# addtt/ladder-vae-pytorch

Hardware: AMD Instinct MI355X
Metric: training images/sec (ELBO step: fwd+bwd+Adamax) (higher is better)
Workload: dtype f32; 1 GPU; CIFAR10-shaped 15-layer LVAE (BASELINE configs[2]): 32x32x3, zdims 32x15, 4 blocks/layer, 64 filters, gated+skip, DMoL-10, dropout 0.2, free bits 1.0; batch_per_gpu=256, global_batch=256, parallelism=dp1, hip_graph=True

## Files before the change

ladder-vae-pytorch_amd/csrc/conv3x3_wino.hip:

```cpp
#include <stdlib.h>
#include <string.h>

#include "bf16_frag.h"
#include "bn_stats.h"
#include "lvae_host.h"

#ifndef LVAE_W1_RING
#define LVAE_W1_RING 3
#endif

namespace lvae {

struct WinoArgs {
  lvae_conv_desc d;
  const float* U;
  int TH, TW, NI, tiles_h, halo_w, halo_h, halo_px, ntn, Npad, tiles_x, wt_per_img, n_wt, Cin;
  uint32_t m_thw, m_per_img, m_halo_w, m_tiles_x, m_wt_per_img, m_tw;
  lvae_bn_fold f;
  int store_pivot;
  const __bf16* g_ws;
  const float* g_bias;
  const float* g_res;
  float* g_ab;
  float* g_out;
// ... 216 lines not shown
      const bool live = hoff[u] != ~0u && 16 * c + hc4 < a.Cin;
      const unsigned off = live ? hoff[u] + 16 * c : 0u;
      if (dbg & 1) hreg[u] = zero4;
      else hreg[u] = *reinterpret_cast<const f32x4*>(d.x + off);
      hlive = live ? hlive | (1u << u) : hlive & ~(1u << u);
    }
  };
  __shared__ __attribute__((aligned(16))) float s_coef[128];
  const bool folded = CIN == 64 && a.f.parts != nullptr;
  const bool bn_in = d.in_scale != nullptr || folded;
  auto store_slice = [&](int c) {
    f32x4 sc = {1.f, 1.f, 1.f, 1.f}, sh = zero4;
    if (bn_in && 16 * c + hc4 < a.Cin) {
      if (folded) {
        sc = *reinterpret_cast<const f32x4*>(s_coef + 16 * c + hc4);
        sh = *reinterpret_cast<const f32x4*>(s_coef + 64 + 16 * c + hc4);
      } else {
        sc = *reinterpret_cast<const f32x4*>(d.in_scale + 16 * c + hc4);
        sh = *reinterpret_cast<const f32x4*>(d.in_shift + 16 * c + hc4);
      }
    }
#pragma unroll
    for (int u = 0; u < SLOTS; ++u) {
      if (hlds[u] >= 0) {
        f32x4 w = zero4;
        if ((hlive >> u) & 1u) {
          w = hreg[u];
          if (bn_in) w = act_fwd4(w * sc + sh, d.in_act);
        }
        *reinterpret_cast<f32x4*>(As + hlds[u] + 16 * c) = w;
      }
    }
  };
  load_slice(0);

  const int ra = wave == 0 ? 0 : (wave == 2 ? 2 : 1);
  const int rb = wave == 0 ? 2 : (wave == 1 ? 2 : (wave == 2 ? 1 : 3));
  const float sgn = wave == 1 ? 1.f : -1.f;
  const float* pa[MT];
  const float* pb[MT];
#pragma unroll
  for (int m = 0; m < MT; ++m) {
    int wt = li + 32 * m;
    if (wt >= a.n_wt) wt = 0;
    const int wimg = fastdiv(wt, a.m_wt_per_img), wr = wt - wimg * a.wt_per_img;
    const int wty = fastdiv(wr, a.m_tiles_x), wtx = wr - wty * a.tiles_x;
    const int pbase = (wimg * a.halo_h + 2 * wty) * a.halo_w + 2 * wtx;
    pa[m] = As + (size_t)(pbase + ra * a.halo_w) * WLDA + (SPL ? 8 : 4) * lh;
    pb[m] = As + (size_t)(pbase + rb * a.halo_w) * WLDA + (SPL ? 8 : 4) * lh;
  }

  f32x16 acc[MT][4][NH];
#pragma unroll
  for (int m = 0; m < MT; ++m)
#pragma unroll
    for (int j = 0; j < 4; ++j)
#pragma unroll
      for (int h = 0; h < NH; ++h)
#pragma unroll
        for (int r = 0; r < 16; ++r) acc[m][j][h][r] = 0.f;

  if (folded) wino_fold_bn<256>(a.f, a.Cin, smem, s_coef, t, bid == 0);
  store_slice(0);
  load_slice(1);
  __syncthreads();
  WINO_STAMP(1);
  if (!SPL) {
    const size_t slab = (size_t)a.Npad * CIN;
    const float* ub = a.U + (size_t)(4 * wave) * slab + ((size_t)lh * a.Npad + co0 + li) * 4;
    const size_t kstep = (size_t)2 * a.Npad * 4;
    f32x4 bf[RING][4][NH];
    auto load_u = [&](int ks, int buf) {
  #pragma unroll
      for (int j = 0; j < 4; ++j)
  #pragma unroll
        for (int h = 0; h < NH; ++h) bf[buf][j][h] = *reinterpret_cast<const f32x4*>(ub + j * slab + ks * kstep + h * 128);
    };
  #pragma unroll
    for (int q = 0; q < RING - 1; ++q) load_u(q, q);

  #pragma unroll
    for (int ks = 0; ks < KSTEPS; ++ks) {
      if (ks + RING - 1 < KSTEPS) load_u(ks + RING - 1, (ks + RING - 1) % RING);
      if (NH == 1) __builtin_amdgcn_sched_barrier(0);
  #pragma unroll
      for (int m = 0; m < MT; ++m) {
        f32x4 tt[4];
  #pragma unroll
        for (int c = 0; c < 4; ++c) {
          const f32x4 da = *reinterpret_cast<const f32x4*>(pa[m] + c * WLDA + ks * 8);
          const f32x4 db = *reinterpret_cast<const f32x4*>(pb[m] + c * WLDA + ks * 8);
  #pragma unroll
          for (int e = 0; e < 4; ++e) tt[c][e] = __builtin_fmaf(sgn, db[e], da[e]);
        }
        f32x4 vv[4];
        vv[0] = tt[0] - tt[2];
        vv[1] = tt[1] + tt[2];
        vv[2] = tt[2] - tt[1];
        vv[3] = tt[1] - tt[3];
  #pragma unroll
        for (int j = 0; j < 4; ++j)
  #pragma unroll
          for (int h = 0; h < NH; ++h)
  #pragma unroll
            for (int e = 0; e < 4; ++e)
              acc[m][j][h] = __builtin_amdgcn_mfma_f32_32x32x2f32(vv[j][e], bf[ks % RING][j][h][e], acc[m][j][h], 0, 0, 0);
      }
      if (NH == 1) __builtin_amdgcn_sched_barrier(0);
      if ((ks & 1) && ks < KSTEPS - 1) {
        const int c = (ks + 1) >> 1;
        store_slice(c);
        if (c + 1 < NSLICE) load_slice(c + 1);
        __syncthreads();
      }
    }
  } else {
    const int NB = a.Npad >> 5;
    const __bf16* u3 = reinterpret_cast<const __bf16*>(a.U) + ((size_t)(co0 >> 5) * 3 * 64 + lane) * 8;
    constexpr int BR = LVAE_W1_RING;
    bf16x8 bq[BR][NH][3];
    auto load_b = [&](int it, int buf) {
      const __bf16* p = u3 + ((dbg & 8) ? (size_t)0 : (size_t)((4 * wave + (it & 3)) * 4 + (it >> 2)) * NB * 1536);
#pragma unroll
      for (int h = 0; h < NH; ++h)
#pragma unroll
        for (int q = 0; q < 3; ++q) bq[buf][h][q] = *reinterpret_cast<const bf16x8*>(p + (h * 3 + q) * 512);
    };
#pragma unroll
    for (int it = 0; it < (BR < 4 * NSLICE ? BR - 1 : BR); ++it) load_b(it, it);
#pragma unroll
    for (int s16 = 0; s16 < NSLICE; ++s16) {
      f32x4 tl[4], th[4];
      if (!(dbg & 2)) {
#pragma unroll
      for (int c = 0; c < 4; ++c) {
        const f32x4 dal = *reinterpret_cast<const f32x4*>(pa[0] + c * WLDA + s16 * 16);
        const f32x4 dah = *reinterpret_cast<const f32x4*>(pa[0] + c * WLDA + s16 * 16 + 4);
        const f32x4 dbl = *reinterpret_cast<const f32x4*>(pb[0] + c * WLDA + s16 * 16);
        const f32x4 dbh = *reinterpret_cast<const f32x4*>(pb[0] + c * WLDA + s16 * 16 + 4);
#pragma unroll
        for (int e = 0; e < 4; ++e) {
          tl[c][e] = __builtin_fmaf(sgn, dbl[e], dal[e]);
          th[c][e] = __builtin_fmaf(sgn, dbh[e], dah[e]);
        }
      }
#pragma unroll
      for (int j = 0; j < 4; ++j) {
        const int it = 4 * s16 + j;
        if (BR < 4 * NSLICE && it + BR - 1 < 4 * NSLICE) load_b(it + BR - 1, (it + BR - 1) % BR);
        const f32x4 vl = j == 0 ? tl[0] - tl[2] : (j == 1 ? tl[1] + tl[2] : (j == 2 ? tl[2] - tl[1] : tl[1] - tl[3]));
        const f32x4 vh = j == 0 ? th[0] - th[2] : (j == 1 ? th[1] + th[2] : (j == 2 ? th[2] - th[1] : th[1] - th[3]));
        bf16x8 af[3];
        if (dbg & 32) {
          af[0] = __builtin_bit_cast(bf16x8, vl);
          af[1] = __builtin_bit_cast(bf16x8, vh);
          af[2] = __builtin_bit_cast(bf16x8, vl + vh);
        } else {
        split_frag<3>(vl, vh, af);
        }
#pragma unroll
        for (int h = 0; h < NH; ++h) acc[0][j][h] = mfma_pieces<3>(af, bq[it % BR][h], acc[0][j][h]);
      }
      } else {
#pragma unroll
        for (int j = 0; j < 4; ++j) {
          const int it = 4 * s16 + j;
          if (BR < 4 * NSLICE && it + BR - 1 < 4 * NSLICE) load_b(it + BR - 1, (it + BR - 1) % BR);
#pragma unroll
          for (int h = 0; h < NH; ++h)
#pragma unroll
            for (int q = 0; q < 3; ++q) acc[0][j][h][q] += (float)bq[it % BR][h][q][0];
        }
      }
      if (s16 < NSLICE - 1) {
        store_slice(s16 + 1);
        if (s16 + 2 < NSLICE) load_slice(s16 + 2);
        __syncthreads();
      }
    }
  }
  WINO_STAMP(2);
  __syncthreads();
  WINO_STAMP(3);
  if (dbg & 16) {
    float keep = 0.f;
#pragma unroll
    for (int j = 0; j < 4; ++j)
#pragma unroll
      for (int h = 0; h < NH; ++h) keep += acc[0][j][h][j + h];
    if (keep == 12345.678f) d.y[t] = 1.f;
    return;
  }

  float* Rs = smem;
#pragma unroll
  for (int m = 0; m < MT; ++m)
#pragma unroll
    for (int h = 0; h < NH; ++h)
#pragma unroll
      for (int r = 0; r < 16; ++r) {
        const int tile = 32 * m + (r & 3) + 8 * (r >> 2) + 4 * lh;
        const float r0 = acc[m][0][h][r] + acc[m][1][h][r] + acc[m][2][h][r];
        const float r1 = acc[m][1][h][r] - acc[m][2][h][r] - acc[m][3][h][r];
        float* o = Rs + (size_t)((wave * 2) * NT + tile) * WLDO + h * 32 + li;
        o[0] = r0;
        o[NT * WLDO] = r1;
      }
  __syncthreads();
  WINO_STAMP(4);
  {
    const int c4 = (t % C4N) * 4, col = co0 + c4;
    f32x4 st1 = zero4, st2 = zero4, piv, bsh, bmu, brs;
    stats_load_coef4(d.stats_pivot, d.Cout, col, d.stats_out != nullptr, d.stats_mode == LVAE_STATS_BN_BWD, piv, bsh, bmu, brs);
    if (col < d.Cout) {
      f32x4 bias = zero4;
      if (d.bias) bias = *reinterpret_cast<const f32x4*>(d.bias + col);
      const int thw = a.TH * a.TW;
      const int nvalid = min(a.NI, d.N - n0) * thw;
      float* yb = d.y + ((size_t)(n0 * d.H + oh0) * d.W) * d.Cout + col;
#pragma unroll
      for (int q = 0; q < QN; ++q) {
        const int p = t / C4N + PG * q;
        if (p < nvalid) {
          const int img = fastdiv(p, a.m_thw), pr = p - img * thw;
          const int oy = fastdiv(pr, a.m_tw), ox = pr - oy * a.TW;
          const int tile = img * a.wt_per_img + (oy >> 1) * a.tiles_x + (ox >> 1);
          const float* rp = Rs + (size_t)((ox & 1) * NT + tile) * WLDO + c4;
          const f32x4 R0 = *reinterpret_cast<const f32x4*>(rp);
          const f32x4 R1 = *reinterpret_cast<const f32x4*>(rp + 2 * NT * WLDO);
          const f32x4 R2 = *reinterpret_cast<const f32x4*>(rp + 4 * NT * WLDO);
          const f32x4 R3 = *reinterpret_cast<const f32x4*>(rp + 6 * NT * WLDO);
          f32x4 v = (oy & 1) ? (R1 - R2 - R3) : (R0 + R1 + R2);
          v = v + bias;
          if (d.out_scale) v = v * *reinterpret_cast<const f32x4*>(d.out_scale + (size_t)(n0 + img) * d.Cout + col);
          v = act_fwd4(v, d.out_act);
          if (!(dbg & 4) || v[0] == 12345.678f) store_wt4(yb + (size_t)p * d.Cout, v);
          if (d.stats_mode == LVAE_STATS_BN_BWD) {
            if (d.stats_out) {
              const f32x4 xv = *reinterpret_cast<const f32x4*>(d.stats_x + (size_t)((n0 * d.H + oh0) * d.W + p) * d.Cout + col);
              stats_bwd_accum4(v, xv, piv, bsh, bmu, brs, d.stats_act, st1, st2);
            }
          } else {
            stats_fwd_accum4(v, piv, st1, st2);
          }
        }
      }
    }
    WINO_STAMP(5);
    if (d.stats_out)
      stats_reduce_groups<PG, CW>(smem, t / C4N, c4, st1, st2, d.stats_out, tm, d.Cout, co0, a.store_pivot && tm == 0, d.stats_pivot,
                                  gridDim.x / a.ntn);
  }
}


#ifndef LVAE_W2_PAIRSPLIT
#define LVAE_W2_PAIRSPLIT 1
#endif

constexpr int W2_LDS_R = 8 * 2 * 32 * WLDO * 4;

template <bool GATE>
__global__ __launch_bounds__(512) void conv3x3_wino2_kernel(WinoArgs a) {
  kernarg_warmup<sizeof(WinoArgs)>();
  constexpr int CIN = 64, WLDA = CIN + 4, NSLICE = CIN / 16, CW = 64, C4N = CW / 4, PG = 512 / C4N, NH = 2;
  extern __shared__ __attribute__((aligned(16))) float smem[];
  float* As = smem;
  const lvae_conv_desc& d = a.d;
  const int t = threadIdx.x, lane = t & 63, wave = __builtin_amdgcn_readfirstlane(t >> 6);
  const int li = lane & 31, lh = lane >> 5;
  const int prow = wave >> 1, jp = wave & 1;
  WINO_STAMP(0);
#ifdef LVAE_WINO_DBG
  constexpr int dbg = LVAE_WINO_DBG;
#else
  constexpr int dbg = 0;
#endif
  int bid = blockIdx.x;
  {
    const int nwg = gridDim.x, xcd = bid & 7, q = nwg >> 3, r = nwg & 7;
    bid = (xcd < r ? xcd * (q + 1) : r * (q + 1) + (xcd - r) * q) + (bid >> 3);
  }
  const int tile_n = bid % a.ntn;
  const int tm = bid / a.ntn;
  const int th_idx = tm % a.tiles_h, ig = tm / a.tiles_h;
  const int n0 = ig * a.NI, oh0 = th_idx * a.TH, co0 = tile_n * CW;
  const f32x4 zero4 = {0.f, 0.f, 0.f, 0.f};

  constexpr int SLOTS = 3;
  const int per_img = a.halo_h * a.halo_w;
  const int hc4 = (t & 3) * 4;
  unsigned hoff[SLOTS];
  int hlds[SLOTS];
#pragma unroll
  for (int u = 0; u < SLOTS; ++u) {
    const int px = (t >> 2) + 128 * u;
    const int img = fastdiv(px, a.m_per_img), r = px - img * per_img;
    const int hy = fastdiv(r, a.m_halo_w), hx = r - hy * a.halo_w;
    const int n = n0 + img, ih = oh0 + hy - 1, iw = hx - 1;
    const bool ok = (n < d.N) & ((unsigned)ih < (unsigned)d.H) & ((unsigned)iw < (unsigned)d.W) & (px < a.halo_px);
    hoff[u] = ok ? (unsigned)(((n * d.H + ih) * d.W + iw) * a.Cin + hc4) : ~0u;
    hlds[u] = px < a.halo_px ? px * WLDA + hc4 : a.halo_px * WLDA + 4 * t;
  }
  __shared__ __attribute__((aligned(16))) float s_coef[128];
  const bool folded = a.f.parts != nullptr;
  const bool bn_in = d.in_scale != nullptr || folded;
  f32x4 hreg[SLOTS];
  unsigned hlive = 0;
  auto load_slice = [&](int c) {
#pragma unroll
    for (int u = 0; u < SLOTS; ++u) {
      const bool live = hoff[u] != ~0u && 16 * c + hc4 < a.Cin;
      const unsigned off = live ? hoff[u] + 16 * c : 0u;
      if (dbg & 1) hreg[u] = zero4;
      else hreg[u] = *reinterpret_cast<const f32x4*>(d.x + off);
      hlive = live ? hlive | (1u << u) : hlive & ~(1u << u);
    }
  };
  auto store_slice = [&](int c) {
    if (bn_in) {
      const int cc = 16 * c + hc4 < a.Cin ? 16 * c + hc4 : 0;
      f32x4 sc, sh;
      if (folded) {
        sc = *reinterpret_cast<const f32x4*>(s_coef + cc);
        sh = *reinterpret_cast<const f32x4*>(s_coef + 64 + cc);
      } else {
        sc = *reinterpret_cast<const f32x4*>(d.in_scale + cc);
        sh = *reinterpret_cast<const f32x4*>(d.in_shift + cc);
      }
#pragma unroll
      for (int u = 0; u < SLOTS; ++u) {
        f32x4 w;
#pragma unroll
        for (int e = 0; e < 4; ++e) w[e] = hreg[u][e] * sc[e] + sh[e];
        w = act_fwd4(w, d.in_act);
        const bool live = (hlive >> u) & 1u;
#pragma unroll
        for (int e = 0; e < 4; ++e) w[e] = live ? w[e] : 0.f;
        *reinterpret_cast<f32x4*>(As + hlds[u] + 16 * c) = w;
      }
    } else {
#pragma unroll
      for (int u = 0; u < SLOTS; ++u) {
        f32x4 w = hreg[u];
        const bool live = (hlive >> u) & 1u;
#pragma unroll
        for (int e = 0; e < 4; ++e) w[e] = live ? w[e] : 0.f;
        *reinterpret_cast<f32x4*>(As + hlds[u] + 16 * c) = w;
      }
    }
  };
  load_slice(0);

  const int ra = prow == 0 ? 0 : (prow == 2 ? 2 : 1);
  const int rb = prow == 0 ? 2 : (prow == 1 ? 2 : (prow == 2 ? 1 : 3));
  const float sgn = prow == 1 ? 1.f : -1.f;
  const float s2 = jp ? -1.f : 1.f;
  const int col0 = jp ? 2 : 0, col1 = jp ? 1 : 2, col2 = jp ? 3 : 1;
  const float* pa[2];
  const float* pb[2];
#pragma unroll
  for (int m = 0; m < 2; ++m) {
    const int wt = li + 32 * m;
    const int wimg = fastdiv(wt, a.m_wt_per_img), wr = wt - wimg * a.wt_per_img;
    const int wty = fastdiv(wr, a.m_tiles_x), wtx = wr - wty * a.tiles_x;
    const int pbase = (wimg * a.halo_h + 2 * wty) * a.halo_w + 2 * wtx;
    pa[m] = As + (size_t)(pbase + ra * a.halo_w) * WLDA + 8 * lh;
    pb[m] = As + (size_t)(pbase + rb * a.halo_w) * WLDA + 8 * lh;
  }

  f32x16 acc[2][2][NH];
#pragma unroll
  for (int m = 0; m < 2; ++m)
#pragma unroll
    for (int j = 0; j < 2; ++j)
#pragma unroll
      for (int h = 0; h < NH; ++h)
#pragma unroll
        for (int r = 0; r < 16; ++r) acc[m][j][h][r] = 0.f;

  if (folded) wino_fold_bn<512>(a.f, a.Cin, smem, s_coef, t, bid == 0);
  store_slice(0);
  load_slice(1);
  __syncthreads();
  WINO_STAMP(1);
  {
    const int NB = a.Npad >> 5;
    const __bf16* u3 = reinterpret_cast<const __bf16*>(a.U) + ((size_t)(co0 >> 5) * 3 * 64 + lane) * 8;
#ifndef LVAE_W2_RING
#define LVAE_W2_RING 2
#endif
    constexpr int BR = LVAE_W2_RING, NIT = 2 * NSLICE;
    bf16x8 bq[BR][NH][3];
    auto load_b = [&](int it, int buf) {
      const __bf16* p = u3 + ((dbg & 8) ? (size_t)0 : (size_t)((4 * prow + 2 * jp + (it & 1)) * 4 + (it >> 1)) * NB * 1536);
#pragma unroll
      for (int h = 0; h < NH; ++h)
#pragma unroll
        for (int q = 0; q < 3; ++q) bq[buf][h][q] = *reinterpret_cast<const bf16x8*>(p + (h * 3 + q) * 512);
    };
#pragma unroll
    for (int it = 0; it < BR - 1; ++it) load_b(it, it);
    auto make_af = [&](const f32x4 (&tl)[2][3], const f32x4 (&th)[2][3], int jj, int m, bf16x8 (&af)[3]) {
      f32x4 vl, vh;
      if (jj == 0) {
#pragma unroll
        for (int e = 0; e < 4; ++e) {
          vl[e] = tl[m][0][e] - tl[m][1][e];
          vh[e] = th[m][0][e] - th[m][1][e];
        }
      } else {
#pragma unroll
        for (int e = 0; e < 4; ++e) {
          vl[e] = __builtin_fmaf(s2, tl[m][2][e], tl[m][1][e]);
          vh[e] = __builtin_fmaf(s2, th[m][2][e], th[m][1][e]);
        }
      }
      if (dbg & 32) {
        af[0] = __builtin_bit_cast(bf16x8, vl);
        af[1] = __builtin_bit_cast(bf16x8, vh);
        af[2] = __builtin_bit_cast(bf16x8, vl + vh);
        return;
      }
#if LVAE_W2_PAIRSPLIT
      split8_3(vl, vh, af);
#else
      split_frag<3>(vl, vh, af);
#endif
    };
#pragma unroll
    for (int s16 = 0; s16 < NSLICE; ++s16) {
      f32x4 tl[2][3], th[2][3];
#pragma unroll
      for (int m = 0; m < 2; ++m)
#pragma unroll
        for (int cc = 0; cc < 3; ++cc) {
          const int c = cc == 0 ? col0 : (cc == 1 ? col1 : col2);
          const f32x4 dal = *reinterpret_cast<const f32x4*>(pa[m] + c * WLDA + s16 * 16);
          const f32x4 dah = *reinterpret_cast<const f32x4*>(pa[m] + c * WLDA + s16 * 16 + 4);
          const f32x4 dbl = *reinterpret_cast<const f32x4*>(pb[m] + c * WLDA + s16 * 16);
          const f32x4 dbh = *reinterpret_cast<const f32x4*>(pb[m] + c * WLDA + s16 * 16 + 4);
#pragma unroll
          for (int e = 0; e < 4; ++e) {
            tl[m][cc][e] = __builtin_fmaf(sgn, dbl[e], dal[e]);
            th[m][cc][e] = __builtin_fmaf(sgn, dbh[e], dah[e]);
          }
        }
      bf16x8 afc[3], afn[3];
      make_af(tl, th, 0, 0, afc);
#pragma unroll
      for (int st = 0; st < 4; ++st) {
        const int jj = st >> 1, m = st & 1, it = 2 * s16 + jj;
        if (m == 0 && it + BR - 1 < NIT) load_b(it + BR - 1, (it + BR - 1) % BR);
        if (st < 3) {
          make_af(tl, th, (st + 1) >> 1, (st + 1) & 1, afn);
        } else if (s16 < NSLICE - 1) {
          store_slice(s16 + 1);
          if (s16 + 2 < NSLICE) load_slice(s16 + 2);
        }
#pragma unroll
        for (int h = 0; h < NH; ++h)
          acc[m][jj][h] = mfma_pieces<3>(afc, bq[it % BR][h], acc[m][jj][h]);
        if (st < 3) {
#pragma unroll
          for (int q = 0; q < 3; ++q) afc[q] = afn[q];
        }
      }
      if (s16 < NSLICE - 1) __syncthreads();
    }
  }
  WINO_STAMP(2);
  __syncthreads();
  WINO_STAMP(3);
  if (dbg & 16) {
    float keep = 0.f;
#pragma unroll
    for (int m = 0; m < 2; ++m)
#pragma unroll
      for (int j = 0; j < 2; ++j)
#pragma unroll
        for (int h = 0; h < NH; ++h) keep += acc[m][j][h][m + j + h];
    if (keep == 12345.678f) d.y[t] = 1.f;
    return;
  }

  float* Rs = smem;
  const int c4 = (t % C4N) * 4, col = co0 + c4;
  f32x4 st1 = zero4, st2 = zero4, piv, bsh, bmu, brs;
  stats_load_coef4(d.stats_pivot, d.Cout, col, d.stats_out != nullptr, d.stats_mode == LVAE_STATS_BN_BWD, piv, bsh, bmu, brs);
  f32x4 bias = zero4;
  if (d.bias && col < d.Cout) bias = *reinterpret_cast<const f32x4*>(d.bias + col);
  const int thw = a.TH * a.TW;
  const int nvalid = min(a.NI, d.N - n0) * thw;
  float* yb = d.y + ((size_t)(n0 * d.H + oh0) * d.W) * d.Cout + col;
#pragma unroll
  for (int m = 0; m < 2; ++m) {
    if (m) {
      WINO_STAMP(5);
      if (GATE) lds_barrier();
      else __syncthreads();
    }
#pragma unroll
    for (int h = 0; h < NH; ++h)
#pragma unroll
      for (int r = 0; r < 16; ++r) {
        const int tile = (r & 3) + 8 * (r >> 2) + 4 * lh;
        const float m0 = acc[m][0][h][r], m1 = acc[m][1][h][r];
        const float r0 = jp ? m0 : m0 + m1;
        const float r1 = jp ? -m0 - m1 : m1;
        float* o = Rs + (size_t)((wave * 2) * 32 + tile) * WLDO + h * 32 + li;
        o[0] = r0;
        o[32 * WLDO] = r1;
      }
    __syncthreads();
    if (m == 0) WINO_STAMP(4); else WINO_STAMP(6);
    f32x4 gy[GATE ? 128 / PG : 1];
    if (GATE) {
#pragma unroll
      for (int q = 0; q < 128 / PG; ++q) gy[q] = zero4;
    }
    const bool want_sx = !GATE && d.stats_out != nullptr && d.stats_mode == LVAE_STATS_BN_BWD && col < d.Cout;
    f32x4 sxr[128 / PG], msk[128 / PG];
#pragma unroll
    for (int q = 0; q < 128 / PG; ++q) {
      const int p = 128 * m + t / C4N + PG * q;
      const int pc = p < nvalid ? p : 0;
      sxr[q] = want_sx ? *reinterpret_cast<const f32x4*>(d.stats_x + (size_t)((n0 * d.H + oh0) * d.W + pc) * d.Cout + col) : zero4;
      const int imgq = fastdiv(pc, a.m_thw);
      msk[q] = (d.out_scale != nullptr && col < d.Cout) ? *reinterpret_cast<const f32x4*>(d.out_scale + (size_t)(n0 + imgq) * d.Cout + col)
                                                         : f32x4{1.f, 1.f, 1.f, 1.f};
    }
    if (col < d.Cout) {
#pragma unroll
      for (int q = 0; q < 128 / PG; ++q) {
        const int p = 128 * m + t / C4N + PG * q;
        if (p < nvalid) {
          const int img = fastdiv(p, a.m_thw), pr = p - img * thw;
          const int oy = fastdiv(pr, a.m_tw), ox = pr - oy * a.TW;
          const int tile = (img * a.wt_per_img + (oy >> 1) * a.tiles_x + (ox >> 1)) & 31;
          const float* rp = Rs + (size_t)((ox & 1) * 32 + tile) * WLDO + c4;
          constexpr int WS = 2 * 32 * WLDO;
          const int i0 = (oy & 1) ? 1 : 0;
          f32x4 Rr[3];
#pragma unroll
          for (int k = 0; k < 3; ++k)
            Rr[k] = *reinterpret_cast<const f32x4*>(rp + (2 * (i0 + k)) * WS) + *reinterpret_cast<const f32x4*>(rp + (2 * (i0 + k) + 1) * WS);
          f32x4 v = (oy & 1) ? (Rr[0] - Rr[1] - Rr[2]) : (Rr[0] + Rr[1] + Rr[2]);
          v = (v + bias) * msk[q];
          v = act_fwd4(v, d.out_act);
          if (!(dbg & 4) || v[0] == 12345.678f) store_wt4(yb + (size_t)p * d.Cout, v);
          if (GATE) {
            gy[q] = v;
          } else if (d.stats_mode == LVAE_STATS_BN_BWD) {
            if (d.stats_out) {
              const f32x4 xv = sxr[q];
              stats_bwd_accum4(v, xv, piv, bsh, bmu, brs, d.stats_act, st1, st2);
            }
          } else {
            stats_fwd_accum4(v, piv, st1, st2);
          }
        }
      }
    }
    if (GATE) {
      constexpr int LDKG = 72, G_PLANE = 128 * LDKG, LDG = 132;
      const size_t grow = (size_t)(n0 * d.H + oh0) * d.W + 128 * m;
      const int prow0 = t / C4N;
      const int gwm = wave >> 1, gwn = wave & 1;
      bf16x8 gqa[4][3], gqb[4][3];
      {
        const __bf16* gws = a.g_ws + lane * 8;
#pragma unroll
        for (int s4 = 0; s4 < 4; ++s4)
#pragma unroll
          for (int k = 0; k < 3; ++k) {
            gqa[s4][k] = *reinterpret_cast<const bf16x8*>(gws + ((size_t)(s4 * 4 + gwn) * 3 + k) * 512);
            gqb[s4][k] = *reinterpret_cast<const bf16x8*>(gws + ((size_t)(s4 * 4 + 2 + gwn) * 3 + k) * 512);
          }
      }
      f32x4 gres[128 / PG];
#pragma unroll
      for (int q = 0; q < 128 / PG; ++q) {
        const int pl = prow0 + PG * q;
        const bool okr = 128 * m + pl < nvalid;
        gres[q] = (a.g_res != nullptr && okr) ? *reinterpret_cast<const f32x4*>(a.g_res + (grow + pl) * 64 + c4) : zero4;
      }
      lds_barrier();
      __bf16* Gs = reinterpret_cast<__bf16*>(smem);
#pragma unroll
      for (int q = 0; q < 128 / PG; ++q) {
        bf16x4 pl3[3];
        split4<3>(gy[q], pl3);
#pragma unroll
        for (int k = 0; k < 3; ++k) *reinterpret_cast<bf16x4*>(Gs + k * G_PLANE + (prow0 + PG * q) * LDKG + c4) = pl3[k];
      }
      lds_barrier();
      f32x16 acca, accb;
#pragma unroll
      for (int r = 0; r < 16; ++r) acca[r] = accb[r] = 0.f;
#pragma unroll
      for (int s4 = 0; s4 < 4; ++s4) {
        bf16x8 af[3];
#pragma unroll
        for (int k = 0; k < 3; ++k) af[k] = *reinterpret_cast<const bf16x8*>(Gs + k * G_PLANE + (gwm * 32 + li) * LDKG + 16 * s4 + 8 * lh);
#pragma unroll
        for (int kk = 0; kk < PieceOrder<3>::N; ++kk) {
          acca = __builtin_amdgcn_mfma_f32_32x32x16_bf16(af[PieceOrder<3>::A[kk]], gqa[s4][PieceOrder<3>::B[kk]], acca, 0, 0, 0);
          accb = __builtin_amdgcn_mfma_f32_32x32x16_bf16(af[PieceOrder<3>::A[kk]], gqb[s4][PieceOrder<3>::B[kk]], accb, 0, 0, 0);
        }
      }
      lds_barrier();
      float* Qs = smem;
#pragma unroll
      for (int r = 0; r < 16; ++r) {
        const int row = gwm * 32 + (r & 3) + 8 * (r >> 2) + 4 * lh;
        Qs[row * LDG + gwn * 32 + li] = acca[r];
        Qs[row * LDG + 64 + gwn * 32 + li] = accb[r];
      }
      lds_barrier();
      f32x4 gba = zero4, gbb = zero4, gpiv = zero4;
      if (a.g_bias) {
        gba = *reinterpret_cast<const f32x4*>(a.g_bias + c4);
        gbb = *reinterpret_cast<const f32x4*>(a.g_bias + 64 + c4);
      }
      if (a.g_stats) gpiv = *reinterpret_cast<const f32x4*>(a.g_pivot + c4);
#pragma unroll
      for (int q = 0; q < 128 / PG; ++q) {
        const int pl = prow0 + PG * q;
        if (128 * m + pl < nvalid) {
          const f32x4 av = *reinterpret_cast<const f32x4*>(Qs + pl * LDG + c4) + gba;
          const f32x4 bv = *reinterpret_cast<const f32x4*>(Qs + pl * LDG + 64 + c4) + gbb;
          if (a.g_ab) {
            store_wt4(a.g_ab + (grow + pl) * 128 + c4, av);
            store_wt4(a.g_ab + (grow + pl) * 128 + 64 + c4, bv);
          }
          f32x4 o = act_fwd4(av, a.g_act);
#pragma unroll
          for (int j = 0; j < 4; ++j) o[j] *= sigmoidf_(bv[j]);
          o += gres[q];
          store_wt4(a.g_out + (grow + pl) * 64 + c4, o);
          stats_fwd_accum4(o, gpiv, st1, st2);
        }
      }
    }
  }
  WINO_STAMP(7);
  float* const so = GATE ? a.g_stats : d.stats_out;
  if (GATE && so != nullptr)
    stats_reduce_groups<PG, CW>(smem, t / C4N, c4, st1, st2, so, tm, 64, 0, tm == 0, a.g_pivot, gridDim.x / a.ntn);
  if (!GATE && d.stats_out)
    stats_reduce_groups<PG, CW>(smem, t / C4N, c4, st1, st2, d.stats_out, tm, d.Cout, co0, a.store_pivot && tm == 0, d.stats_pivot,
                                gridDim.x / a.ntn);
}


static int wino_kpad(const lvae_conv_desc* d) { return d->C1 <= 64 ? 64 : 128; }
static bool kpad_is64(const lvae_conv_desc* d) { return d->C1 <= 64; }

static bool wino_tile_for(const lvae_conv_desc* d, int budget, int max_halo, int& TH, int& NI) {
  TH = 0;
  for (int c = 2; c <= d->H; c += 2)
    if (d->H % c == 0 && c * d->W <= budget) TH = c;
  if (TH == 0) return false;
  NI = TH < d->H ? 1 : budget / (TH * d->W);
  if (NI < 1) NI = 1;
  if (NI > d->N) NI = d->N;
  return NI * (TH + 2) * (d->W + 2) <= max_halo;
}

static bool wino_narrow(const lvae_conv_desc* d, int TH, int NI) {
  static const int narrow_tiles = (int)tune("LVAE_WINO_NARROW_TILES", 256);
  return kpad_is64(d) && ((d->N + NI - 1) / NI) * (d->H / TH) < narrow_tiles;
}

static bool wino_split_form(const lvae_conv_desc* d) {
  if (d->precision != LVAE_PREC_F32 || !kpad_is64(d) || d->form == LVAE_FORM_F32_MFMA) return false;
  int TH, NI;
  return wino_tile_for(d, 128, 256, TH, NI) && !wino_narrow(d, TH, NI);
}

static size_t conv3x3_wino_workspace(const lvae_conv_desc* d) {
  const int ntn = (d->Cout + 63) / 64;
  if (wino_split_form(d)) return (size_t)16 * 4 * (2 * ntn) * 3 * 1024;
  return (size_t)16 * ntn * 64 * wino_kpad(d) * sizeof(float);
}

static bool conv3x3_wino_eligible(const lvae_conv_desc* d) {
  static const bool off = tune("LVAE_DISABLE_WINO", 0) != 0;
  if (off) return false;
  const int Cin = d->C1;
  if (d->KH != 3 || d->KW != 3 || d->stride != 1 || d->pad != 1 || d->x2 != nullptr || d->OH != d->H || d->OW != d->W) return false;
  if (Cin < 36 || Cin > 128 || Cin % 4 != 0 || d->Cout % 4 != 0 || (d->H & 1) || (d->W & 1) || d->W > 128) return false;
  if (!al16_or_null(d->x) || !al16_or_null(d->y) || !al16_or_null(d->bias) || !al16_or_null(d->in_scale) || !al16_or_null(d->in_shift) || !al16_or_null(d->out_scale)) return false;
  const int64_t M = (int64_t)d->N * d->H * d->W;
  static const int64_t min_m = tune("LVAE_WINO_MIN_M", 256 * 64);
  if (M < min_m || M * 128 >= ((int64_t)1 << 31)) return false;
  return true;
}

struct WinoTile {
  int TH, NI, mt;
};

static bool wino2_tile(const lvae_conv_desc* d, int& TH, int& NI) {
  static const bool off = tune("LVAE_DISABLE_WINO2", 0) != 0;
  if (off || !wino_split_form(d) || !wino_tile_for(d, 256, 384, TH, NI)) return false;
  const int tiles_x = d->W / 2, wt_per_img = (TH / 2) * tiles_x;
  if (NI * wt_per_img != 64 || 32 % tiles_x != 0) return false;
  if (wt_per_img % 32 != 0 && 32 % wt_per_img != 0) return false;
  const int64_t groups = (int64_t)((d->N + NI - 1) / NI) * (d->H / TH) * ((d->Cout + 63) / 64);
  return groups >= 256;
}

static bool wino_tile(const lvae_conv_desc* d, WinoTile& w) {
  int TH, NI;
  if (wino2_tile(d, TH, NI)) {
    w = WinoTile{TH, NI, 2};
    return true;
  }
  if (!wino_tile_for(d, 128, 256, TH, NI)) return false;
  w = WinoTile{TH, NI, 1};
  return true;
}

static size_t wino_lds_bytes(const lvae_conv_desc* d, const WinoTile& w) {
  size_t lds = (size_t)w.NI * (w.TH + 2) * (d->W + 2) * (wino_kpad(d) + 4) * sizeof(float);
  const size_t lds_r = w.mt == 2 ? (size_t)W2_LDS_R : (size_t)4 * 2 * 32 * WLDO * sizeof(float);
  return lds < lds_r ? lds_r : lds;
}

static bool wino_folds(const lvae_conv_desc* d, const WinoTile& w) {
  static const bool off = tune("LVAE_DISABLE_WINO_FOLD", 0) != 0;
  if (off || d->C1 > 64) return false;
  const bool narrow = w.mt == 1 && wino_narrow(d, w.TH, w.NI);
  const int64_t wgs = (int64_t)((d->N + w.NI - 1) / w.NI) * (d->H / w.TH) * (narrow ? (d->Cout + 31) / 32 : (d->Cout + 63) / 64);
  static const int64_t max_wgs = tune("LVAE_WINO_FOLD_MAX_WGS", 512);
  return wgs <= max_wgs;
}

bool conv3x3_wino_plan(const lvae_conv_desc* d, bool assume_ws, ConvPlan& p) {
  if (!conv3x3_wino_eligible(d)) return false;
  const size_t ws = conv3x3_wino_workspace(d);
  if (!assume_ws && (d->workspace == nullptr || (size_t)d->workspace_bytes < ws || !al16_or_null(d->workspace))) return false;
  WinoTile w;
  if (!wino_tile(d, w) || wino_lds_bytes(d, w) > 159 * 1024) return false;
  p = ConvPlan{};
  p.variant = wino_split_form(d) ? LVAE_VARIANT_WINO_SIX : LVAE_VARIANT_WINO_F32;
  p.rows = ((d->N + w.NI - 1) / w.NI) * (d->H / w.TH);
  p.folds = wino_folds(d, w);
  p.workspace = ws;
  return true;
}

int conv3x3_wino2_gate_rows(const lvae_conv_desc* d) {
  if (d->C1 != 64 || d->Cout != 64 || d->out_act != LVAE_ACT_NONE || d->gather != LVAE_GATHER_CONV) return 0;
  ConvPlan p;
  WinoTile w;
  if (!conv3x3_wino_plan(d, false, p) || (d->in_fold != nullptr && !p.folds) || !wino_tile(d, w) || w.mt != 2) return 0;
  return p.rows;
}

static int wino_launch(const lvae_conv_desc* d, const lvae_rb_ext* gate, hipStream_t s) {
  WinoTile wtile;
  wino_tile(d, wtile);
  const int Cin = d->C1;
  WinoArgs a;
  a.d = *d;
  const int TH = wtile.TH, NI = wtile.NI, mt = wtile.mt;
  const bool split = wino_split_form(d);
  a.TH = TH;
  a.TW = d->W;
  a.NI = NI;
  a.tiles_h = d->H / TH;
  a.halo_h = TH + 2;
  a.halo_w = d->W + 2;
  a.halo_px = NI * a.halo_h * a.halo_w;
  a.tiles_x = d->W / 2;
  a.wt_per_img = (TH / 2) * a.tiles_x;
  a.n_wt = NI * a.wt_per_img;
  a.Npad = (d->Cout + 63) / 64 * 64;
  const bool narrow = mt == 1 && wino_narrow(d, TH, NI);
  a.ntn = narrow ? (d->Cout + 31) / 32 : (d->Cout + 63) / 64;
  a.m_thw = fastdiv_magic(TH * d->W);
  a.m_tw = fastdiv_magic(d->W);
  a.m_per_img = fastdiv_magic(a.halo_h * a.halo_w);
  a.m_halo_w = fastdiv_magic(a.halo_w);
  a.m_tiles_x = fastdiv_magic(a.tiles_x);
  a.m_wt_per_img = fastdiv_magic(a.wt_per_img);
  const int kpad = wino_kpad(d);
  a.Cin = Cin;
  const size_t lds = wino_lds_bytes(d, wtile);
  const bool folds = wino_folds(d, wtile);
  a.f = lvae_bn_fold{};
  if (d->in_fold != nullptr) a.f = *d->in_fold;
  a.d.in_fold = nullptr;
  a.store_pivot = folds && d->stats_out != nullptr && d->stats_mode == LVAE_STATS_BN_FWD;
  a.g_ws = nullptr;
  a.g_bias = a.g_res = a.g_pivot = nullptr;
  a.g_ab = a.g_out = a.g_stats = nullptr;
  a.g_act = 0;
  if (gate != nullptr) {
    a.g_ws = static_cast<const __bf16*>(gate->gate_ws);
    a.g_bias = gate->gate_bias;
    a.g_res = gate->res;
    a.g_ab = gate->ab;
    a.g_out = gate->out;
    a.g_stats = gate->out_stats;
    a.g_pivot = gate->out_stats_pivot;
    a.g_act = gate->act;
  }
  float* U = static_cast<float*>(d->workspace);
  a.U = U;
  const int Npad = a.Npad;
  if (!d->workspace_ready) {
    hipLaunchKernelGGL(wino_weight_kernel, dim3((Npad * kpad + 255) / 256), dim3(256), 0, s, d->w, d->w_stap, d->w_sk, d->w_sn, Cin,
                       kpad, d->Cout, Npad, d->gather == LVAE_GATHER_TRANSPOSED ? 1 : 0, U, split ? 1 : 0);
    LVAE_LAUNCH_CHECK("wino_weight");
  }
  const int img_groups = (d->N + NI - 1) / NI;
  const dim3 grid(img_groups * a.tiles_h * a.ntn);
  const char* name = "conv3x3_wino";
  if (mt == 2 && gate != nullptr) return launch_lds<conv3x3_wino2_kernel<true>>(name, grid, dim3(512), lds, 159 * 1024, s, a);
  if (mt == 2) return launch_lds<conv3x3_wino2_kernel<false>>(name, grid, dim3(512), lds, 159 * 1024, s, a);
  if (split) return launch_lds<conv3x3_wino_kernel<64, 2, 1, true>>(name, grid, dim3(256), lds, 80 * 1024, s, a);
  if (narrow) return launch_lds<conv3x3_wino_kernel<64, 1, 1, false>>(name, grid, dim3(256), lds, 80 * 1024, s, a);
  if (kpad == 64) return launch_lds<conv3x3_wino_kernel<64, 2, 1, false>>(name, grid, dim3(256), lds, 80 * 1024, s, a);
  return launch_lds<conv3x3_wino_kernel<128, 2, 1, false>>(name, grid, dim3(256), lds, 159 * 1024, s, a);
}

int conv3x3_wino_launch(const lvae_conv_desc* d, hipStream_t s) { return wino_launch(d, nullptr, s); }

int conv3x3_wino2_gate_launch(const lvae_conv_desc* d, const lvae_rb_ext* gate, hipStream_t s) { return wino_launch(d, gate, s); }

}

using namespace lvae;

extern "C" size_t lvae_conv2d_prepare_entry_bytes(void) { return sizeof(WinoPrepEntry); }

extern "C" int lvae_conv2d_prepare_entry(const lvae_conv_desc* d, void* entry) {
  LVAE_REQUIRE(d && entry, LVAE_EINVAL, "lvae_conv2d_prepare_entry: null pointer");
  ConvPlan pos;
  if (!conv3x3_pos_plan(d, pos)) {
    const int form = conv3x3_bf16_form(d);
    if (form != 0) {
      LVAE_REQUIRE(d->workspace && (size_t)d->workspace_bytes >= conv3x3_bf16_workspace(d, form) && al16_or_null(d->workspace), LVAE_EINVAL,
                   "lvae_conv2d_prepare_entry: no scratch for the pre-split weights");
      conv3x3_bf16_prep_entry(d, form, entry);
      return 0;
    }
  }
  LVAE_REQUIRE(conv3x3_wino_eligible(d) && d->workspace && (size_t)d->workspace_bytes >= conv3x3_wino_workspace(d) &&
                   al16_or_null(d->workspace),
               LVAE_EINVAL, "lvae_conv2d_prepare_entry: descriptor has no weight pre-transform (lvae_conv2d_workspace(d) == 0) or no scratch");
  WinoPrepEntry e;
  e.w = d->w;
  e.U = static_cast<float*>(d->workspace);
  e.stap = d->w_stap;
  e.sk = d->w_sk;
  e.sn = d->w_sn;
  e.K = d->C1;
  e.N = d->Cout;
  e.Npad = (d->Cout + 63) / 64 * 64;
  e.flip = d->gather == LVAE_GATHER_TRANSPOSED ? 1 : 0;
  e.Kpad = wino_kpad(d);
  e.pad_ = wino_split_form(d) ? 16 : 0;
  memcpy(entry, &e, sizeof(e));
  return 0;
}

extern "C" int lvae_conv2d_prepare_weights(const void* entries, int32_t n, int32_t max_cout, void* stream) {
  LVAE_REQUIRE(entries && n > 0 && n < 65536 && max_cout > 0, LVAE_EINVAL, "lvae_conv2d_prepare_weights: bad arguments");
  const int npad = (max_cout + 63) / 64 * 64;
  hipLaunchKernelGGL(wino_weight_batched_kernel, dim3((npad * 128 + 255) / 256, n), dim3(256), 0, (hipStream_t)stream,
                     static_cast<const WinoPrepEntry*>(entries));
  LVAE_LAUNCH_CHECK("wino_weight_batched");
  return conv3x3_bf16_prepare_batched(entries, n, npad, (hipStream_t)stream);
}

#if defined(LVAE_WINO_DBG) && (LVAE_WINO_DBG & 64)
extern "C" int lvae_debug_wino_stamps(void* host_out, size_t bytes) {
  return (int)hipMemcpyFromSymbol(host_out, HIP_SYMBOL(lvae::g_wino_stamps), bytes < sizeof(lvae::g_wino_stamps) ? bytes : sizeof(lvae::g_wino_stamps));
}
#endif
```

ladder-vae-pytorch_amd/csrc/lvae_common.h:

```cpp
#pragma once
#include <hip/hip_runtime.h>
#include <stdint.h>
#include <stdio.h>
#include <stdlib.h>

#include <atomic>

#include "../../include/lvae_hip.h"

namespace lvae {

typedef float f32x16 __attribute__((ext_vector_type(16)));
typedef float f32x4 __attribute__((ext_vector_type(4)));
typedef float f32x2 __attribute__((ext_vector_type(2)));

void set_error(const char* fmt, ...);

inline int debug_phase_switch(const char* name) {
#ifdef LVAE_PHASE_DEBUG
  const char* v = getenv(name);
  return v ? atoi(v) : 0;
#else
  (void)name;
  return 0;
#endif
}

inline int64_t tune(const char* name, int64_t dflt) {
#ifdef LVAE_TUNING_ENV
  const char* v = getenv(name);
  return v ? atoll(v) : dflt;
#else
  (void)name;
  return dflt;
#endif
}

#define LVAE_REQUIRE(cond, code, ...)  \
  do {                                 \
    if (!(cond)) {                     \
      lvae::set_error(__VA_ARGS__);    \
      return (code);                   \
    }                                  \
  } while (0)

#define LVAE_LAUNCH_CHECK(name)                                        \
  do {                                                                 \
    hipError_t e__ = hipGetLastError();                                \
    if (e__ != hipSuccess) {                                           \
      lvae::set_error("%s: launch failed: %s", name, hipGetErrorString(e__)); \
      return (int)e__;                                                 \
    }                                                                  \
  } while (0)

inline bool al16(const void* p) { return (reinterpret_cast<uintptr_t>(p) & 15) == 0; }
inline bool al16_or_null(const void* p) { return p == nullptr || al16(p); }

#ifndef LVAE_WT_STORES
#define LVAE_WT_STORES 1
#endif
__device__ __forceinline__ void store_wt4(float* p, f32x4 v) {
#if LVAE_WT_STORES
  asm volatile("global_store_dwordx4 %0, %1, off sc1\n\ts_nop 1" : : "v"(p), "v"(v) : "memory");
#else
  *reinterpret_cast<f32x4*>(p) = v;
#endif
}

__device__ __forceinline__ void lds_barrier() { asm volatile("s_waitcnt lgkmcnt(0)\n\ts_barrier" ::: "memory"); }

#ifndef LVAE_KERNARG_WARM
#define LVAE_KERNARG_WARM 1
#endif
template <int BYTES>
__device__ __forceinline__ void kernarg_warmup() {
#if LVAE_KERNARG_WARM
  const char* kp = (const char*)__builtin_amdgcn_kernarg_segment_ptr();
  constexpr int NL = (BYTES + 63) / 64;
  unsigned ka[NL];
#pragma unroll
  for (int i = 0; i < NL; ++i) asm volatile("s_load_dword %0, %1, %2" : "=s"(ka[i]) : "s"(kp), "n"(i * 64) : "memory");
  asm volatile("s_waitcnt lgkmcnt(0)" ::: "memory");
#pragma unroll
  for (int i = 0; i < NL; ++i) asm volatile("" ::"s"(ka[i]));
#endif
}

__device__ __forceinline__ float byte_to_unit(unsigned v) { return __fdiv_rn((float)v, 255.0f); }

constexpr float kSeluAlpha = 1.6732632423543772848170429916717f;
constexpr float kSeluScale = 1.0507009873554804934193349852946f;

__device__ __forceinline__ float act_fwd(float x, int act) {
  switch (act) {
    case LVAE_ACT_ELU: return x > 0.f ? x : __expf(x) - 1.f;
    case LVAE_ACT_RELU: return x > 0.f ? x : 0.f;
    case LVAE_ACT_LEAKYRELU: return x > 0.f ? x : 0.01f * x;
    case LVAE_ACT_SELU: return kSeluScale * (x > 0.f ? x : kSeluAlpha * (__expf(x) - 1.f));
    default: return x;
  }
}

__device__ __forceinline__ f32x4 act_fwd4(f32x4 v, int act) {
  if (act == LVAE_ACT_NONE) return v;
  if (act == LVAE_ACT_ELU) {
#pragma unroll
    for (int j = 0; j < 4; ++j) v[j] = v[j] > 0.f ? v[j] : __expf(v[j]) - 1.f;
    return v;
  }
#pragma unroll
  for (int j = 0; j < 4; ++j) v[j] = act_fwd(v[j], act);
  return v;
}

__device__ __forceinline__ f32x16 act_fwd16(f32x16 v, int act) {
  if (act == LVAE_ACT_NONE) return v;
  if (act == LVAE_ACT_ELU) {
#pragma unroll
    for (int j = 0; j < 16; ++j) v[j] = v[j] > 0.f ? v[j] : __expf(v[j]) - 1.f;
    return v;
  }
#pragma unroll
  for (int j = 0; j < 16; ++j) v[j] = act_fwd(v[j], act);
  return v;
}

__device__ __forceinline__ float act_grad(float x, int act) {
  switch (act) {
    case LVAE_ACT_ELU: return x > 0.f ? 1.f : __expf(x);
    case LVAE_ACT_RELU: return x > 0.f ? 1.f : 0.f;
    case LVAE_ACT_LEAKYRELU: return x > 0.f ? 1.f : 0.01f;
    case LVAE_ACT_SELU: return kSeluScale * (x > 0.f ? 1.f : kSeluAlpha * __expf(x));
    default: return 1.f;
  }
}

__device__ __forceinline__ f32x4 act_grad4(f32x4 u, int act) {
  f32x4 r;
  if (act == LVAE_ACT_ELU) {
#pragma unroll
    for (int j = 0; j < 4; ++j) r[j] = u[j] > 0.f ? 1.f : __expf(u[j]);
    return r;
  }
#pragma unroll
  for (int j = 0; j < 4; ++j) r[j] = act_grad(u[j], act);
  return r;
}

__device__ __forceinline__ float act_grad_from_out(float y, int act) {
  switch (act) {
    case LVAE_ACT_ELU: return y > 0.f ? 1.f : y + 1.f;
    case LVAE_ACT_RELU: return y > 0.f ? 1.f : 0.f;
    case LVAE_ACT_LEAKYRELU: return y > 0.f ? 1.f : 0.01f;
    case LVAE_ACT_SELU: return y > 0.f ? kSeluScale : y + kSeluScale * kSeluAlpha;
    default: return 1.f;
  }
}

__device__ __forceinline__ float sigmoidf_(float x) { return __builtin_amdgcn_rcpf(1.f + __expf(-x)); }

__device__ __forceinline__ float softplusf_(float x) { return x > 20.f ? x : log1pf(expf(x)); }

__device__ __forceinline__ float normal_kl(float qmu, float qlv, float pmu, float plv) {
  const float qs = expf(0.5f * qlv), ps = expf(0.5f * plv);
  const float r = qs / ps, vr = r * r;
  const float t = (qmu - pmu) / ps;
  return 0.5f * (vr + t * t - 1.f - logf(vr));
}

constexpr float kLogSqrt2Pi = 0.91893853320467274178f;
__device__ __forceinline__ float normal_logprob(float z, float mu, float lv) {
  const float sd = expf(0.5f * lv);
  const float d = z - mu;
  return -(d * d) / (2.f * sd * sd) - logf(sd) - kLogSqrt2Pi;
}

__device__ __forceinline__ float anneal_beta(const int64_t* step, int64_t anneal_steps) {
  if (anneal_steps <= 0) return 1.f;
  const double r = fmin(fmax((double)step[0] / (double)anneal_steps, 0.0), 1.0);
  return (float)(0.0 + (1.0 - 0.0) * r);
}

__device__ __forceinline__ float wave_sum(float v) {
#pragma unroll
  for (int o = 32; o > 0; o >>= 1) v += __shfl_xor(v, o, 64);
  return v;
}

__device__ __forceinline__ float block_sum_256(float v, float* red) {
  v = wave_sum(v);
  __syncthreads();
  if ((threadIdx.x & 63) == 0) red[threadIdx.x >> 6] = v;
  __syncthreads();
  return red[0] + red[1] + red[2] + red[3];
}

inline uint32_t fastdiv_magic(int d) { return d <= 1 ? 0u : (uint32_t)((((uint64_t)1 << 32) + d - 1) / (uint64_t)d); }
__device__ __forceinline__ int fastdiv(int n, uint32_t magic) { return magic ? (int)__umulhi((uint32_t)n, magic) : n; }

inline int grid_for(int64_t work_items, int per_block, int cap = 256 * 8) {
  int64_t g = (work_items + per_block - 1) / per_block;
  if (g < 1) g = 1;
  if (g > cap) g = cap;
  return (int)g;
}

}
```

Baseline: 9466 images/s.

## Prefetch Winograd epilogue operands early and replace syncthreads with LDS-only barriers

The Winograd conv epilogue now issues its global loads (bias, stats pivots, residual or stats_x rows, out_scale masks, gate weights and gate bias) before the LDS scatter of accumulators. It pins them in registers with empty asm so their latency overlaps the scatter and barrier, and the second half's rows are prefetched during the first half. It also replaces __syncthreads with lds_barrier, which waits only on LDS counters, and stages the gate bias and pivot through an enlarged s_coef shared buffer. In exchange, register pressure rises from holding two halves of rows, and unused loads go through a dummy pointer instead of being predicated off.

```diff
diff --git a/ladder-vae-pytorch_amd/csrc/conv3x3_wino.hip b/ladder-vae-pytorch_amd/csrc/conv3x3_wino.hip
--- a/ladder-vae-pytorch_amd/csrc/conv3x3_wino.hip
+++ b/ladder-vae-pytorch_amd/csrc/conv3x3_wino.hip
@@ -542,7 +542,7 @@
     hoff[u] = ok ? (unsigned)(((n * d.H + ih) * d.W + iw) * a.Cin + hc4) : ~0u;
     hlds[u] = px < a.halo_px ? px * WLDA + hc4 : a.halo_px * WLDA + 4 * t;
   }
-  __shared__ __attribute__((aligned(16))) float s_coef[128];
+  __shared__ __attribute__((aligned(16))) float s_coef[GATE ? 256 : 128];
   const bool folded = a.f.parts != nullptr;
   const bool bn_in = d.in_scale != nullptr || folded;
   f32x4 hreg[SLOTS];
@@ -726,19 +726,82 @@
 
   float* Rs = smem;
   const int c4 = (t % C4N) * 4, col = co0 + c4;
-  f32x4 st1 = zero4, st2 = zero4, piv, bsh, bmu, brs;
-  stats_load_coef4(d.stats_pivot, d.Cout, col, d.stats_out != nullptr, d.stats_mode == LVAE_STATS_BN_BWD, piv, bsh, bmu, brs);
-  f32x4 bias = zero4;
-  if (d.bias && col < d.Cout) bias = *reinterpret_cast<const f32x4*>(d.bias + col);
+  f32x4 st1 = zero4, st2 = zero4;
   const int thw = a.TH * a.TW;
   const int nvalid = min(a.NI, d.N - n0) * thw;
   float* yb = d.y + ((size_t)(n0 * d.H + oh0) * d.W) * d.Cout + col;
+  const int prow0 = t / C4N;
+  const size_t grow0 = (size_t)(n0 * d.H + oh0) * d.W;
+  const int gwm = wave >> 1, gwn = wave & 1;
+  const bool want_sx = !GATE && d.stats_out != nullptr && d.stats_mode == LVAE_STATS_BN_BWD && col < d.Cout;
+  const bool want_aux = GATE ? a.g_res != nullptr : want_sx;
+  const float* const dummy = d.x + c4;
+  auto pick = [&](bool want, const float* p) {
+    const float* r = want ? p : dummy;
+    asm("" : "+v"(r));
+    return (const __attribute__((address_space(1))) f32x4*)(uintptr_t)r;
+  };
+  const bool want_piv = !GATE && d.stats_out != nullptr && col < d.Cout, want_bwd = want_piv && d.stats_mode == LVAE_STATS_BN_BWD;
+  const bool want_bias = d.bias != nullptr && col < d.Cout;
+  f32x4 piv = zero4, bsh = zero4, bmu = zero4, brs = zero4;
+  if (!GATE) {
+    piv = *pick(want_piv, d.stats_pivot + col);
+    bsh = *pick(want_bwd, d.stats_pivot + d.Cout + col);
+    bmu = *pick(want_bwd, d.stats_pivot + 2 * d.Cout + col);
+    brs = *pick(want_bwd, d.stats_pivot + 3 * d.Cout + col);
+  }
+  f32x4 bias = *pick(want_bias, d.bias + col);
+  const bool want_msk = d.out_scale != nullptr && col < d.Cout;
+  f32x4 msk[2][128 / PG], aux[2][128 / PG];
+  int rpc[2][128 / PG], rimg[2][128 / PG];
+  auto index_rows = [&](int m) {
+#pragma unroll
+    for (int q = 0; q < 128 / PG; ++q) {
+      const int p = 128 * m + prow0 + PG * q;
+      rpc[m][q] = p < nvalid ? p : 0;
+      rimg[m][q] = fastdiv(rpc[m][q], a.m_thw);
+    }
+  };
+  index_rows(0);
+  if (!GATE) index_rows(1);
+  auto load_rows = [&](int m) {
+#pragma unroll
+    for (int q = 0; q < 128 / PG; ++q) {
+      const int pc = rpc[m][q];
+      const float* ap = GATE ? a.g_res + (grow0 + pc) * 64 + c4 : d.stats_x + (size_t)((n0 * d.H + oh0) * d.W + pc) * d.Cout + col;
+      aux[m][q] = *pick(want_aux, ap);
+      const int imgq = rimg[m][q];
+      msk[m][q] = *pick(want_msk, d.out_scale + (size_t)(n0 + imgq) * d.Cout + col);
+    }
+  };
+  auto close_rows = [&](int m) {
+#pragma unroll
+    for (int q = 0; q < 128 / PG; ++q) {
+      close_load(aux[m][q]);
+      close_load(msk[m][q]);
+      const bool keep = want_aux && (!GATE || 128 * m + prow0 + PG * q < nvalid);
+#pragma unroll
+      for (int e = 0; e < 4; ++e) {
+        aux[m][q][e] = keep ? aux[m][q][e] : 0.f;
+        msk[m][q][e] = want_msk ? msk[m][q][e] : 1.f;
+      }
+    }
+  };
+  bf16x8 gqa[GATE ? 4 : 1][3], gqb[GATE ? 4 : 1][3];
+  const bool want_gb = GATE && a.g_bias != nullptr, want_gp = GATE && a.g_stats != nullptr;
+  f32x4 gba0 = *pick(want_gb, a.g_bias + c4);
+  f32x4 gbb0 = *pick(want_gb, a.g_bias + 64 + c4);
+  f32x4 gpiv0 = *pick(want_gp, a.g_pivot + c4);
+  load_rows(0);
 #pragma unroll
   for (int m = 0; m < 2; ++m) {
     if (m) {
       WINO_STAMP(5);
-      if (GATE) lds_barrier();
-      else __syncthreads();
+      lds_barrier();
+      if (GATE) {
+        index_rows(1);
+        load_rows(1);
+      }
     }
 #pragma unroll
     for (int h = 0; h < NH; ++h)
@@ -752,28 +815,80 @@
         o[0] = r0;
         o[32 * WLDO] = r1;
       }
-    __syncthreads();
+    if (m == 0) {
+      if (GATE) {
+        const __bf16* gws = a.g_ws + lane * 8;
+#pragma unroll
+        for (int s4 = 0; s4 < 4; ++s4)
+#pragma unroll
+          for (int k = 0; k < 3; ++k) {
+            gqa[s4][k] = *reinterpret_cast<const bf16x8*>(gws + ((size_t)(s4 * 4 + gwn) * 3 + k) * 512);
+            gqb[s4][k] = *reinterpret_cast<const bf16x8*>(gws + ((size_t)(s4 * 4 + 2 + gwn) * 3 + k) * 512);
+          }
+      } else {
+        load_rows(1);
+      }
+    }
+    lds_barrier();
     if (m == 0) WINO_STAMP(4); else WINO_STAMP(6);
+    if (m == 0) {
+      if (!GATE) {
+        close_load(piv);
+        close_load(bsh);
+        close_load(bmu);
+        close_load(brs);
+        close_load(bias);
+#pragma unroll
+        for (int e = 0; e < 4; ++e) {
+          piv[e] = want_piv ? piv[e] : 0.f;
+          bsh[e] = want_bwd ? bsh[e] : piv[e];
+          bmu[e] = want_bwd ? bmu[e] : piv[e];
+          brs[e] = want_bwd ? brs[e] : piv[e];
+          bias[e] = want_bias ? bias[e] : 0.f;
+        }
+      }
+      close_rows(0);
+      if (GATE) {
+        close_load(bias);
+        close_load(gba0);
+        close_load(gbb0);
+        close_load(gpiv0);
+#pragma unroll
+        for (int e = 0; e < 4; ++e) {
+          bias[e] = want_bias ? bias[e] : 0.f;
+          gba0[e] = want_gb ? gba0[e] : 0.f;
+          gbb0[e] = want_gb ? gbb0[e] : 0.f;
+          gpiv0[e] = want_gp ? gpiv0[e] : 0.f;
+        }
+        if (prow0 == 0) {
+          *reinterpret_cast<f32x4*>(s_coef + c4) = bias;
+          *reinterpret_cast<f32x4*>(s_coef + 64 + c4) = gba0;
+          *reinterpret_cast<f32x4*>(s_coef + 128 + c4) = gbb0;
+          *reinterpret_cast<f32x4*>(s_coef + 192 + c4) = gpiv0;
+        }
+#pragma unroll
+        for (int s4 = 0; s4 < 4; ++s4)
+#pragma unroll
+          for (int k = 0; k < 3; ++k) {
+            close_load(gqa[s4][k]);
+            close_load(gqb[s4][k]);
+          }
+      } else {
+        close_rows(1);
+      }
+    } else if (GATE) {
+      close_rows(1);
+    }
     f32x4 gy[GATE ? 128 / PG : 1];
     if (GATE) {
 #pragma unroll
       for (int q = 0; q < 128 / PG; ++q) gy[q] = zero4;
     }
-    const bool want_sx = !GATE && d.stats_out != nullptr && d.stats_mode == LVAE_STATS_BN_BWD && col < d.Cout;
-    f32x4 sxr[128 / PG], msk[128 / PG];
-#pragma unroll
-    for (int q = 0; q < 128 / PG; ++q) {
-      const int p = 128 * m + t / C4N + PG * q;
-      const int pc = p < nvalid ? p : 0;
-      sxr[q] = want_sx ? *reinterpret_cast<const f32x4*>(d.stats_x + (size_t)((n0 * d.H + oh0) * d.W + pc) * d.Cout + col) : zero4;
-      const int imgq = fastdiv(pc, a.m_thw);
-      msk[q] = (d.out_scale != nullptr && col < d.Cout) ? *reinterpret_cast<const f32x4*>(d.out_scale + (size_t)(n0 + imgq) * d.Cout + col)
-                                                         : f32x4{1.f, 1.f, 1.f, 1.f};
-    }
+    if (GATE && m == 1) bias = *reinterpret_cast<const f32x4*>(s_coef + c4);
     if (col < d.Cout) {
 #pragma unroll
       for (int q = 0; q < 128 / PG; ++q) {
-        const int p = 128 * m + t / C4N + PG * q;
+        const int p = 128 * m + prow0 + PG * q;
         if (p < nvalid) {
           const int img = fastdiv(p, a.m_thw), pr = p - img * thw;
           const int oy = fastdiv(pr, a.m_tw), ox = pr - oy * a.TW;
@@ -786,14 +901,14 @@
           for (int k = 0; k < 3; ++k)
             Rr[k] = *reinterpret_cast<const f32x4*>(rp + (2 * (i0 + k)) * WS) + *reinterpret_cast<const f32x4*>(rp + (2 * (i0 + k) + 1) * WS);
           f32x4 v = (oy & 1) ? (Rr[0] - Rr[1] - Rr[2]) : (Rr[0] + Rr[1] + Rr[2]);
-          v = (v + bias) * msk[q];
+          v = (v + bias) * msk[m][q];
           v = act_fwd4(v, d.out_act);
           if (!(dbg & 4) || v[0] == 12345.678f) store_wt4(yb + (size_t)p * d.Cout, v);
           if (GATE) {
             gy[q] = v;
           } else if (d.stats_mode == LVAE_STATS_BN_BWD) {
             if (d.stats_out) {
-              const f32x4 xv = sxr[q];
+              const f32x4 xv = aux[m][q];
               stats_bwd_accum4(v, xv, piv, bsh, bmu, brs, d.stats_act, st1, st2);
             }
           } else {
@@ -804,27 +919,7 @@
     }
     if (GATE) {
       constexpr int LDKG = 72, G_PLANE = 128 * LDKG, LDG = 132;
-      const size_t grow = (size_t)(n0 * d.H + oh0) * d.W + 128 * m;
-      const int prow0 = t / C4N;
-      const int gwm = wave >> 1, gwn = wave & 1;
-      bf16x8 gqa[4][3], gqb[4][3];
-      {
-        const __bf16* gws = a.g_ws + lane * 8;
-#pragma unroll
-        for (int s4 = 0; s4 < 4; ++s4)
-#pragma unroll
-          for (int k = 0; k < 3; ++k) {
-            gqa[s4][k] = *reinterpret_cast<const bf16x8*>(gws + ((size_t)(s4 * 4 + gwn) * 3 + k) * 512);
-            gqb[s4][k] = *reinterpret_cast<const bf16x8*>(gws + ((size_t)(s4 * 4 + 2 + gwn) * 3 + k) * 512);
-          }
-      }
-      f32x4 gres[128 / PG];
-#pragma unroll
-      for (int q = 0; q < 128 / PG; ++q) {
-        const int pl = prow0 + PG * q;
-        const bool okr = 128 * m + pl < nvalid;
-        gres[q] = (a.g_res != nullptr && okr) ? *reinterpret_cast<const f32x4*>(a.g_res + (grow + pl) * 64 + c4) : zero4;
-      }
+      const size_t grow = grow0 + 128 * m;
       lds_barrier();
       __bf16* Gs = reinterpret_cast<__bf16*>(smem);
 #pragma unroll
@@ -858,12 +953,8 @@
         Qs[row * LDG + 64 + gwn * 32 + li] = accb[r];
       }
       lds_barrier();
-      f32x4 gba = zero4, gbb = zero4, gpiv = zero4;
-      if (a.g_bias) {
-        gba = *reinterpret_cast<const f32x4*>(a.g_bias + c4);
-        gbb = *reinterpret_cast<const f32x4*>(a.g_bias + 64 + c4);
-      }
-      if (a.g_stats) gpiv = *reinterpret_cast<const f32x4*>(a.g_pivot + c4);
+      const f32x4 gba = *reinterpret_cast<const f32x4*>(s_coef + 64 + c4), gbb = *reinterpret_cast<const f32x4*>(s_coef + 128 + c4);
+      const f32x4 gpiv = *reinterpret_cast<const f32x4*>(s_coef + 192 + c4);
 #pragma unroll
       for (int q = 0; q < 128 / PG; ++q) {
         const int pl = prow0 + PG * q;
@@ -877,7 +968,7 @@
           f32x4 o = act_fwd4(av, a.g_act);
 #pragma unroll
           for (int j = 0; j < 4; ++j) o[j] *= sigmoidf_(bv[j]);
-          o += gres[q];
+          o += aux[m][q];
           store_wt4(a.g_out + (grow + pl) * 64 + c4, o);
           stats_fwd_accum4(o, gpiv, st1, st2);
         }
diff --git a/ladder-vae-pytorch_amd/csrc/lvae_common.h b/ladder-vae-pytorch_amd/csrc/lvae_common.h
--- a/ladder-vae-pytorch_amd/csrc/lvae_common.h
+++ b/ladder-vae-pytorch_amd/csrc/lvae_common.h
@@ -69,6 +69,9 @@
 
 __device__ __forceinline__ void lds_barrier() { asm volatile("s_waitcnt lgkmcnt(0)\n\ts_barrier" ::: "memory"); }
 
+template <class T>
+__device__ __forceinline__ void close_load(T& v) { asm volatile("" : "+v"(v)); }
+
 #ifndef LVAE_KERNARG_WARM
 #define LVAE_KERNARG_WARM 1
 #endif
```

Measured after the change: 9621 images/s, median of 6. 1.6% higher.
